# ltatzel/PyTorchHessianFree

Hardware: AMD Instinct MI355X
Metric: GGN-matvecs/sec (damped operator calls inside the PCG loop) (higher is better)
Workload: dtype f32

## Files before the change

include/hf_pcg.h:

```cpp
#ifndef HF_PCG_H
#define HF_PCG_H

#include <stdint.h>

#ifdef __cplusplus
extern "C" {
#endif

#define HF_ABI_VERSION 13

enum hf_dtype { HF_F32 = 0, HF_F64 = 1 };

enum hf_reason {
  HF_RUNNING = 0,
  HF_REASON_MARTENS = 1,
  HF_REASON_MAXITER = 2,
  HF_REASON_DIVERGED = 3,
  HF_REASON_TOL = 4
};

enum hf_precond {
  HF_M_NONE = 0,
  HF_M_DIAG = 1,
  HF_M_EXTERNAL = 2
// ... 229 lines not shown
int hf_maxpool_forward_nhwc(void* out, void* out2, int64_t out2_ld, void* idx, const void* x, int64_t n,
                            int64_t h, int64_t w, int64_t oh, int64_t ow, int64_t c, int64_t kh, int64_t kw,
                            int64_t stride_h, int64_t stride_w, int64_t pad_h, int64_t pad_w, int dtype,
                            void* stream);
int hf_maxpool_adjoint_nhwc(void* g, const void* gy_a, int a_splits, int64_t a_slab, const void* gy_b,
                            int b_splits, int64_t b_slab, const void* idx, int64_t n, int64_t h, int64_t w,
                            int64_t oh, int64_t ow, int64_t c, int64_t kh, int64_t kw, int64_t stride_h,
                            int64_t stride_w, int64_t pad_h, int64_t pad_w, int dtype, void* stream);
int hf_linear_ce_head(void* g_feat, void* g_w, void* g_b, const void* t_feat, const void* feat, const void* w,
                      const void* v_w, const void* v_b, const void* p, double scale, int64_t rows,
                      int64_t features, int64_t classes, int dtype, void* stream);
int hf_linear_ce_head_slabs(int64_t rows);
int hf_pool_ce_head(void* g, void* jv_out, const void* t, const void* p, double scale, int64_t n, int64_t hw,
                    int64_t k, int dtype, void* stream);

typedef struct hf_comm hf_comm_t;
int hf_comm_unique_id(char* out128);
int hf_comm_create(hf_comm_t** out, const char* id128, int nranks, int rank);
int hf_comm_destroy(hf_comm_t* c);
int hf_allreduce_sum(hf_comm_t* c, void* buf, int64_t n, int dtype, void* stream);
int hf_allreduce_sum_multi(hf_comm_t* c, void* const* bufs, const int64_t* ns, int count, int dtype,
                           void* stream);

#ifdef __cplusplus
}
#endif
#endif
```

pytorchhessianfree_amd/_lib.py:

```python

import ctypes
import os

import torch

_HERE = os.path.dirname(os.path.abspath(__file__))
LIB_PATH = os.environ.get("HF_PCG_LIB") or os.path.join(_HERE, "csrc", "libhfpcg.so")

HF_F32, HF_F64 = 0, 1
ABI_VERSION = 13
HF_ERR_ARG = -1
HF_M_NONE, HF_M_DIAG, HF_M_EXTERNAL = 0, 1, 2
REASONS = {
    1: "Convergence (Martens)",
    2: "Number of iterations",
    3: "Divergence",
    4: "Convergence (tolerances)",
}

c_void_p, c_int, c_int64, c_double = (
    ctypes.c_void_p,
    ctypes.c_int,
    ctypes.c_int64,
    ctypes.c_double,
)
# ... 75 lines not shown
                                                  c_int, c_void_p]),
    "hf_chan_affine_bwd": (c_int, [c_void_p] * 11 + [c_int64, c_int64, c_int64, c_int, c_int, c_void_p]),
    "hf_conv2d_nhwc": (c_int, [c_int, c_void_p, c_void_p, c_void_p] + [c_int64] * 12
                       + [c_void_p, c_int64, c_void_p, c_int64, c_int, c_int, c_void_p]),
    "hf_conv2d_nhwc_backward": (c_int, [c_void_p] * 5 + [c_int64] * 11
                                + [c_void_p, c_int64, c_void_p, c_int64, c_int, c_int, c_void_p]),
    "hf_conv2d_nhwc_plan": (c_int, [c_int] + [c_int64] * 11 + [c_int]),
    "hf_conv2d_nhwc_slabs": (c_int, [c_int, c_void_p, c_void_p, c_void_p] + [c_int64] * 14
                             + [c_int, c_int64, c_int, c_void_p]),
    "hf_conv2d_nhwc_slabs_unpack": (c_int, [c_void_p, c_void_p, c_void_p] + [c_int64] * 13 + [c_int, c_int64, c_void_p,
                                            ctypes.POINTER(c_void_p)] + [ctypes.POINTER(c_int64)] * 6
                                    + [c_int, c_int, c_void_p]),
    "hf_conv2d_nhwc_group_slabs": (c_int, [c_void_p, c_int, c_int, c_void_p]),
    "hf_conv2d_nhwc_dw_slabs": (c_int, [c_void_p, c_void_p, c_int, c_void_p]),
    "hf_chan_affine_pair": (c_int, [c_void_p, c_int, c_void_p]),
    "hf_chan_affine_bwd_pair": (c_int, [c_void_p, c_int, c_void_p]),
    "hf_conv2d_nhwc_backward_slabs": (c_int, [c_void_p] * 5 + [c_int64] * 11
                                      + [c_int, c_int64, c_int, c_int64, c_int, c_void_p]),
    "hf_chan_affine_ex": (c_int, [c_void_p] * 10 + [c_int, c_int64, c_int64, c_int64, c_int, c_int64, c_int64,
                                                     c_int, c_int64, c_int, c_void_p]),
    "hf_chan_affine_bwd_ex": (c_int, [c_void_p] * 5 + [c_int, c_int64, c_void_p, c_int, c_int64] + [c_void_p] * 5
                              + [c_int64, c_int64, c_int64, c_int, c_int, c_int, c_void_p]),
    "hf_chan_affine_train": (c_int, [c_void_p] * 8 + [c_int, c_void_p, c_void_p, c_double, c_void_p, c_void_p]
                             + [c_int64] * 5 + [c_int, c_int64, c_int, c_void_p]),
    "hf_conv2d_nhwc_group_slabs_bnsum": (c_int, [c_void_p, c_int, c_void_p, c_int, c_void_p]),
    "hf_bn_forward_train": (c_int, [c_void_p, c_void_p, c_int64, c_void_p, c_void_p, c_int] + [c_void_p] * 4
                            + [c_double] * 3 + [c_void_p] * 3 + [c_int64, c_int, c_int64, c_int64, c_int, c_void_p]),
    "hf_chan_affine_train_pair": (c_int, [c_void_p, c_int, c_void_p]),
    "hf_bn_train_hessian_coeffs": (c_int, [c_void_p] * 5 + [c_int, c_void_p, c_void_p, c_int] + [c_void_p] * 5
                                   + [c_double, c_int64, c_int, c_void_p]),
# ... 285 lines not shown
    check(
        lib.hf_pack_ex(c_void_p(dst.data_ptr()), ptrs, numels, perm, spl, lv, n, float(scale), int(mode),
                       dtype_code(dst.dtype), current_stream_ptr(dst.device)),
        "hf_pack_ex")
    return dst


class AffineProblem(ctypes.Structure):

    _fields_ = ([("out", c_void_p)] + [(nm, c_void_p) for nm in ("a", "x", "mean", "rstd", "w", "q", "r", "add",
                                                                   "mask_src")]
                + [("relu_self", c_int)] + [(nm, c_int64) for nm in ("n", "c", "hw", "out_ld", "add_ld")]
                + [("a_splits", c_int), ("a_slab", c_int64)])


class BnAdjointProblem(ctypes.Structure):

    _fields_ = ([(nm, c_void_p) for nm in ("gx", "gw", "gb", "gres", "gy")] + [("gy_splits", c_int), ("gy_slab", c_int64),
                                                                                 ("gy2", c_void_p), ("gy2_splits", c_int),
                                                                                 ("gy2_slab", c_int64)]
                + [(nm, c_void_p) for nm in ("x", "mean", "rstd", "w", "mask_src")]
                + [(nm, c_int64) for nm in ("n", "c", "hw")] + [("row_blocks", c_int)])


class AffineTrainProblem(ctypes.Structure):

    _fields_ = ([("out", c_void_p)] + [(nm, c_void_p) for nm in ("a", "x", "mean", "rstd", "w", "part_x", "part_1")]
                + [("nparts", c_int), ("vq", c_void_p), ("vr", c_void_p), ("count", ctypes.c_double),
                   ("add", c_void_p), ("mask_src", c_void_p)]
                + [(nm, c_int64) for nm in ("n", "c", "hw", "out_ld")] + [("a_splits", c_int), ("a_slab", c_int64)])
# ... 85 lines not shown
```

pytorchhessianfree_amd/config.py:

```python

import os
import shutil
import tempfile

_SHIPPED_DB = os.path.join(os.path.dirname(os.path.abspath(__file__)), "miopen_db")
_state = {"done": False, "settings": None}


def user_db_dir():
    base = os.environ.get("XDG_CACHE_HOME") or os.path.join(os.path.expanduser("~"), ".cache")
    return os.path.join(base, "pytorchhessianfree_amd", "miopen_db")


def _seed_user_db(dst):
    os.makedirs(dst, exist_ok=True)
    for name in sorted(os.listdir(_SHIPPED_DB)):
        src, out = os.path.join(_SHIPPED_DB, name), os.path.join(dst, name)
        if not os.path.isfile(src) or os.path.exists(out):
            continue
        fd, tmp = tempfile.mkstemp(dir=dst, prefix=name + ".")
        os.close(fd)
        try:
            shutil.copyfile(src, tmp)
            os.replace(tmp, out)
# ... 52 lines not shown
                "tests/test_optimizer_gpu.py::test_deterministic_mode_products_are_bitwise_repeatable"),
    "HF_NHWC_FIND": ("", "1: keep MIOpen's find step for NHWC problems (used once to produce the shipped records)",
                     "tests/test_host_logic_cpu.py::test_configure_is_explicit_and_idempotent"),
    "HF_SESSION": ("1", "0: no persistent engine session (engine + graphs rebuilt per step)",
                   "tests/test_session_gpu.py::test_session_equals_generic_path_and_is_faster_to_restart"),
    "HF_SESSION_VERIFY": ("", "1: re-verify the session against the model's own forward pass every step",
                          "tests/test_session_gpu.py::test_session_is_reverified_against_the_models_own_forward"),
    "HF_SESSION_VERIFY_EVERY": ("16", "every how many steps the session is re-verified",
                                "tests/test_session_gpu.py::test_session_is_reverified_against_the_models_own_forward"),
    "HF_ACC_SESSION": ("1", "0: acc_step on the generic accumulation",
                       "tests/test_acc_session_gpu.py::test_acc_step_train_mode_batchnorm_session_equals_generic_accumulation"),
    "HF_GRAPH_VERIFY": ("first", "always / never: replay check of a freshly captured product graph",
                        "tests/test_optimizer_gpu.py::test_graphed_operator_refuses_a_replay_that_differs_from_the_eager_product"),
    "HF_FUSE_ITERATION": ("1", "0: product, K1, K2, K3 as separate launches (no iteration graph)",
                          "tests/test_engine_gpu.py::test_solve_as_one_graph_per_iteration_equals_separate_launches"),
    "HF_BN_EPILOGUE": ("1", "0: train-mode tangent partial sums by the reduction launch, not the convolution's epilogue",
                       "tests/test_engine_gpu.py::test_train_mode_prologue_form_variants_agree_and_state_is_independent_of_the_first_use_check"),
    "HF_BN_TRAIN_PAIR": ("1", "0: a downsample block's two train-mode units in launches of their own",
                         "tests/test_engine_gpu.py::test_train_mode_prologue_form_variants_agree_and_state_is_independent_of_the_first_use_check"),
    "HF_CHUNKED_ALLREDUCE": ("auto", "0 / 1: force the single-graph resp. the two-phase data-parallel product",
                             "tests/test_distributed_gpu.py::test_step_two_ranks_engine_session_equals_cpu_whole_batch"),
    "HF_DIRECT_RCCL": ("1", "0: every collective through torch.distributed (no communicator of the package's own)",
                       "tests/test_distributed_gpu.py::test_bench_ladder_reaches_the_plainest_rung"),
    "HF_TEST_DP_FAULT": ("", "test hook: hang / raise / mismatch[:not_plain] -- the last rank misbehaves in a data-parallel "
                             "session product (session._inject_fault)",
                         "tests/test_distributed_gpu.py::test_bench_ladder_falls_past_a_rung_that_hangs"),
    "HF_PCG_BLOCKS": ("0", "workgroups of the PCG vector kernels (0: 2 per CU); must agree on all ranks",
                      "tests/test_cg_gpu.py::test_kernel_grid_override_gives_the_same_solve"),
    "HF_PCG_LIB": ("", "path of another build of libhfpcg.so (tuning variants)",
                   "tests/test_boundary.py::test_alternate_library_path"),
# ... 7 lines not shown
```

pytorchhessianfree_amd/csrc/build.py:

```python

import os
import subprocess
import sys

HERE = os.path.dirname(os.path.abspath(__file__))
ROOT = os.path.dirname(os.path.dirname(HERE))
SOURCES = [os.path.join(HERE, f) for f in ("hf_pcg.hip", "hf_pack.hip", "hf_bn.hip", "hf_conv.hip", "hf_head.hip",
                                           "hf_rccl.hip")]
HDR = os.path.join(ROOT, "include", "hf_pcg.h")
HDRS_SHARED = [os.path.join(HERE, f) for f in ("hf_common.h", "hf_unpack.h")]
OUT = os.path.join(HERE, "libhfpcg.so")

FLAGS = [
    "--offload-arch=gfx950",
    "-O3",
    "-std=c++17",
    "-fPIC",
    "-ffp-contract=off",
    "-fno-fast-math",
    "-Wall",
    "-Wno-unused-function",
]


# ... 37 lines not shown
```

pytorchhessianfree_amd/engine/adjoint.py:

```python

import os

import torch

from .. import _lib
from .common import _cl, _pair, _ptr


class _AdjointSweep:
    def _bn_adjoint_pair_train(self, u1, srcs1, u2, srcs2):
        self._bn_adjoint_pair(u1, srcs1, u2, srcs2, train=True)
        arr = (_lib.AffineTrainProblem * 2)()
        for q, u in zip(arr, (u1, u2)):
            self._affine_train_problem(q, u, u.ga, 0, u.g, 1, 0, u.gw, u.gb, u.rb, None, None, None)
        _lib.check(_lib.load().hf_chan_affine_train_pair(_lib.ctypes.cast(arr, _lib.c_void_p), _lib.HF_F32,
                                                         _lib.current_stream_ptr(self.dev)), "hf_chan_affine_train_pair")

    def _bn_adjoint_pair(self, u1, srcs1, u2, srcs2, train=False):
        arr = (_lib.BnAdjointProblem * 2)()
        for q, u, srcs in zip(arr, (u1, u2), (srcs1, srcs2)):
            if not 1 <= len(srcs) <= 2:
                raise RuntimeError(f"{u.name}: {len(srcs)} consumers")
            (a, sa, la) = srcs[0]
            (b, sb, lb) = srcs[1] if len(srcs) == 2 else (None, 1, 0)
            n, k, oh, ow = u.a.shape
            q.gx, q.gw, q.gb, q.gres = (None if train else u.ga.data_ptr()), u.gw.data_ptr(), u.gb.data_ptr(), u.g.data_ptr()
            q.gy, q.gy_splits, q.gy_slab = a.data_ptr(), sa, la
            q.gy2, q.gy2_splits, q.gy2_slab = (None if b is None else b.data_ptr()), sb, lb
            q.x, q.mean, q.rstd, q.w = u.a.data_ptr(), u.mean.data_ptr(), u.rstd.data_ptr(), u.bn.weight.data_ptr()
            q.mask_src = u.y.data_ptr() if u.relu else None
            q.n, q.c, q.hw, q.row_blocks = n, k, oh * ow, u.rb
        _lib.check(_lib.load().hf_chan_affine_bwd_pair(_lib.ctypes.cast(arr, _lib.c_void_p), _lib.HF_F32,
                                                       _lib.current_stream_ptr(self.dev)), "hf_chan_affine_bwd_pair")

    def _adjoint_unit(self, u, srcs):
        second = self._second and u.bn is not None
        self._bn_adjoint(u, srcs, reduce_only=second and u.train)
        if not second:
            self._conv_adjoint(u)
            return
        lib, st = _lib.load(), _lib.current_stream_ptr(self.dev)
        n, k, oh, ow = u.a.shape
        v = self._v
        v_gamma = v[self._offs[u.pg]: self._offs[u.pg] + k] if u.pg is not None else self._zeros(k)
        if not self._extras_parallel:
            self._hessian_extras(u)
        if u.train:
            rb = u.rb
            tx, t1, nparts_t = u.tsums
            _lib.check(lib.hf_bn_train_hessian_coeffs(
# ... 62 lines not shown

    def _adjoint_blocks(self, g_last, first=None, last_block=0, incoming=None):
        group = self._grouping()
        tail = self.tail
        if incoming is None:
            incoming = {id(tail): [(g_last, 1, 0)]}
        pool_srcs = None
        first = len(self.blocks) - 1 if first is None else first
        stop = max(last_block, self.dead_blocks)
        for bi in range(first, stop - 1, -1):
            chain, ds, _x = self.blocks[bi]
            head, last = chain[0], chain[-1]
            for k in range(len(chain) - 1, -1, -1):
                u = chain[k]
                if k == 0 and ds is not None and group:
                    if u.rb > 1 and ds.rb > 1 and not u.train and not ds.train:
                        self._bn_adjoint_pair(u, incoming.pop(id(u)), ds, [(last.g, 1, 0)])
                    elif u.rb > 1 and ds.rb > 1 and self._train_pair_ok(u, ds):
                        self._bn_adjoint_pair_train(u, incoming.pop(id(u)), ds, [(last.g, 1, 0)])
                    else:
                        self._bn_adjoint(u, incoming.pop(id(u)))
                        self._bn_adjoint(ds, [(last.g, 1, 0)])
                    if u.no_dgrad:
                        _lib.conv_group_slabs(
                            [(2, u.wbuf, u.x, u.ga, u.geo, u.sW, 0, 0), (2, ds.wbuf, ds.x, ds.ga, ds.geo, ds.sW, 0, 0)],
                            self.dev)
                    else:
                        _lib.conv_group_slabs(
                            [(1, u.dbuf, u.ga, u.wT, u.geo, u.sD, 0, 0), (2, u.wbuf, u.x, u.ga, u.geo, u.sW, 0, 0),
                             (1, ds.dbuf, ds.ga, ds.wT, ds.geo, ds.sD, 0, 0),
# ... 124 lines not shown
```

pytorchhessianfree_amd/engine/buffers.py:

```python

import os

import torch
from torch import nn

from .. import _lib
from .common import _Unsupported, _flat_view, _live_taps, _pair, _ptr


class _Buffers:
    ADJ_BYTES_PER_WG = 32768
    def _plan(self, direction, u, forward=False):
        n, c, h, w = u.x.shape
        k, _, r, s = u.conv.weight.shape
        cin = 2 * c if (direction == 0 and not forward) else c
        sp = _lib.load().hf_conv2d_nhwc_plan(direction, n, h, w, cin, k, r, s, u.conv.stride[0], u.conv.stride[1],
                                             u.conv.padding[0], u.conv.padding[1],
                                             0)
        if sp < 1:
            raise _Unsupported(f"{u.name}: convolution geometry refused ({sp})")
        return sp

    def _allocate(self):
        dev, f32 = self.dev, torch.float32
        cl = torch.channels_last

        def nhwc(shape):
            return torch.empty(shape, dtype=f32, device=dev).contiguous(memory_format=cl)

        self._nhwc = nhwc
        self.x_in = nhwc(self._in_shape)
        if self.pool_args is not None:
            self.pool_out = nhwc(self.pool_out.shape)
        for u in self.units:
            u.a, u.y = nhwc(u.a.shape), nhwc(u.y.shape)
            if u.train:
                u.rstd_version = None
            elif u.bn is not None:
                u.rstd = torch.rsqrt(u.bn.running_var + u.bn.eps)
                u.rstd_version = u.bn.running_var._version
        tails = {id(c[-1]): c[0] for c, _, _ in self.blocks}
        for u in self.units:
            u.x = self.x_in if u.src == "input" else self.pool_out if u.src == "pool" else u.src.y
            if u.res_unit is not None:
                u.res = u.res_unit.y
            elif u.res_identity:
                u.res = tails[id(u)].x
            else:
                u.res = None
        xcats = {}
        self._tangent_slots = {}
        for u in self.units:
            n, c, h, w = u.x.shape
            k, _, r, s = u.conv.weight.shape
            if u.im2col:
                if c * r * s > 256:
                    raise _Unsupported(f"{u.name}: too many taps for the im2col formulation")
                oh, ow = u.a.shape[2], u.a.shape[3]
                j = c * r * s
                u.cols = torch.empty((n, oh * ow, j), dtype=f32, device=dev)
                u.geo = (n * oh * ow, 1, 1, j, k, 1, 1, (1, 1), (0, 0))
                jp = -(-j // 4) * 4
                u.cols_pad = torch.zeros((n, oh * ow, jp), dtype=f32, device=dev)
                u.geo_w = (n * oh * ow, 1, 1, jp, k, 1, 1, (1, 1), (0, 0))
# ... 11 lines not shown
                u.wcat = torch.zeros((k, 2 * c, r, s), dtype=f32, device=dev).contiguous(memory_format=cl)
                u.wT = torch.empty((c, r, s, k), dtype=f32, device=dev)
                u.live = _live_taps(h, w, r, s, u.conv.stride, u.conv.padding)
                if u.pw is not None:
                    self._tangent_slots[id(u)] = (self._offs[u.pw], u.wcat, c, u.live)
            oh, ow = u.a.shape[2], u.a.shape[3]
            u.rows, u.cout = n * oh * ow, k
            if u.im2col:
                u.sT = u.sF = self._plan_stem(0, u.geo)
                u.sW = self._plan_stem(2, u.geo_w)
                u.sD = 0
            else:
                u.sT, u.sW = self._plan(0, u), self._plan(2, u)
                u.sD = 0 if (u.first or u.no_dgrad or u.dead) else self._plan(1, u)
                u.sF = self._plan(0, u, forward=True)
            u.tbuf = torch.empty((max(u.sT, u.sF), u.rows * k), dtype=f32, device=dev)
            u.nW = u.sW * (2 if (self.hessian and not u.first) else 1)
            u.nD = u.sD * (2 if self.hessian else 1)
            u.wbuf = torch.zeros((u.nW, u.conv.weight.numel()), dtype=f32, device=dev)
            if u.sD:
                u.dbuf = torch.empty((u.nD, u.x.numel()), dtype=f32, device=dev)
            if self.hessian:
                u.ga1 = torch.empty_like(u.a)
                if u.bn is not None:
                    u.g1 = torch.empty_like(u.a)
                    u.gah = torch.empty_like(u.a)
                if u.sD:
                    u.vT = torch.zeros((c, r, s, k), dtype=f32, device=dev)
            u.g = torch.empty_like(u.a) if u.needs_g else None
            u.ga = torch.empty_like(u.a)
            u.rb = 1
            if k % 4 == 0 and k // 4 <= 256 and u.rows >= 64:
                rp = 256 // (k // 4)
                tgt = min(1024, max(64, u.a.numel() * 4 // self.ADJ_BYTES_PER_WG))
                per = max(rp, -(-u.rows // tgt))
                u.rb = -(-u.rows // per)
                if u.rb < 2:
                    u.rb = 1
            u.gw_rows = u.rb * (2 if (self.hessian and u.bn is not None) else 1)
            if self.hessian and u.train:
                u.gw_rows += 1
            u.gw = torch.empty((u.gw_rows, k), dtype=f32, device=dev)
            u.gb = torch.empty((u.rb, k), dtype=f32, device=dev)
            if u.train:
                if not (k % 4 == 0 and k // 4 <= 256):
                    raise _Unsupported(f"{u.name}: train-mode BatchNorm over {k} channels (the prologue form takes "
                                       "multiples of 4 up to 1024)")
                u.stat_part = torch.empty((u.rb, 2, k), dtype=torch.float64, device=dev)
                tp_rows = -(-u.rows // 64) * u.sT
                u.epi = (not u.im2col and not u.first and hasattr(u, "xcat")
                         and tp_rows <= 256
                         and os.environ.get("HF_BN_EPILOGUE", "1") != "0")
                if self.hessian:
# ... 161 lines not shown
```

pytorchhessianfree_amd/engine/common.py:

```python

import os

import torch

from .. import _lib

_P = _lib.c_void_p


def _ptr(t):
    return _P(t.data_ptr()) if t is not None else None


def _same(a, b):
    return a is not None and b is not None and a.data_ptr() == b.data_ptr() and a.shape == b.shape


def _cl(t):
    return t.contiguous(memory_format=torch.channels_last)


class _Unit:

    def __init__(self, name, conv, bn):
        self.name, self.conv, self.bn = name, conv, bn
        self.rstd = None
        self.first = False
        self.needs_g = True
        self.im2col = False
        self.train = False
        self.mean_t = None
        self.epi = self.tsum = False
        self.res_unit = None
        self.res_identity = False
        self.consumers = 0
        self.src = None
        self.dead = False
        self.no_dgrad = False

    @property
    def mean(self):
        if self.train:
            return self.mean_t
        return self.bn.running_mean if self.bn is not None else None

    @property
    def scale(self):
        return self.bn.weight if self.bn is not None else None

    @property
    def shift(self):
        return self.bn.bias if self.bn is not None else self.conv.bias

# ... 84 lines not shown
    if p0.dtype != torch.float32 or not p0.is_cuda:
        return None
    base, off = p0.data_ptr(), 0
    for p in params:
        if not p.is_contiguous() or p.data_ptr() != base + 4 * off or p.dtype != torch.float32:
            return None
        off += p.numel()
    try:
        if p0.untyped_storage().nbytes() < 4 * (p0.storage_offset() + n) or base % 16:
            return None
        return p0.detach().as_strided((n,), (1,), p0.storage_offset())
    except Exception:
        return None


def _live_taps(h, w, r, s, stride, padding):
    if r * s > 16:
        return 0
    oh = (h + 2 * padding[0] - r) // stride[0] + 1
    ow = (w + 2 * padding[1] - s) // stride[1] + 1
    rows = [any(0 <= o * stride[0] - padding[0] + i < h for o in range(oh)) for i in range(r)]
    cols = [any(0 <= o * stride[1] - padding[1] + j < w for o in range(ow)) for j in range(s)]
    mask = sum(1 << (i * s + j) for i in range(r) for j in range(s) if rows[i] and cols[j])
    return 0 if mask == (1 << (r * s)) - 1 else mask
```

pytorchhessianfree_amd/engine/tangent.py:

```python

import os

import torch

from .. import _lib
from .common import _ptr


class _TangentSweep:
    def _bn_tangent(self, u, v, add, add_ld):
        n, k, oh, ow = u.a.shape
        vg = v[self._offs[u.pg]: self._offs[u.pg] + k] if u.pg is not None else None
        vb = v[self._offs[u.pb]: self._offs[u.pb] + k] if u.pb is not None else None
        if u.train:
            lib, st = _lib.load(), _lib.current_stream_ptr(self.dev)
            px, p1, nparts = u.gw, u.gb, u.rb
            if self.hessian:
                px, p1 = u.hx, u.h1
                _lib.check(lib.hf_chan_affine_bwd_ex(
                    None, _ptr(u.gw[u.rb:]), None, None, _ptr(u.tbuf), u.sT, u.tbuf.shape[1], None, 1, 0, _ptr(u.g1),
                    _ptr(self._zeros(k)), _ptr(u.rstd), None, None, n, k, oh * ow, 1, u.rb, _lib.HF_F32, st),
                    "hf_chan_affine_bwd_ex")
            if u.tsum:
                px, p1, nparts = u.tpx, u.tp1, u.tp1.shape[0]
# ... 77 lines not shown
            sums = [(u.a, u.mean, u.rstd, u.tpx, u.tp1) if u.epi else None for u in units]
            if _lib.conv_group_slabs_bnsum(probs, sums, self.dev):
                for u in units:
                    u.tsum = u.epi
                return
            for u in units:
                u.epi = False
        for u in units:
            u.tsum = False
        if len(units) == 1:
            u = units[0]
            self._conv_slabs(0, u.tbuf, u.xcat, u.wcat, self._tgeo(u), u.sT)
        else:
            _lib.conv_group_slabs(probs, self.dev)

    def _tangent_blocks(self, v):
        group = self._grouping()
        for chain, ds, _x in self.blocks[self.dead_blocks:]:
            head = chain[0]
            paired = False
            if ds is not None and group:
                self._tangent_convs([ds, head])
                alone = head.res_unit is None and not head.res_identity and len(chain) > 1
                paired = alone and not head.train and not ds.train
                if paired:
                    self._bn_tangent_pair(ds, head, v)
                elif alone and self._train_pair_ok(ds, head) and ds.tsum and head.tsum:
                    self._bn_tangent_pair_train(ds, head, v)
                    paired = True
                else:
                    self._bn_tangent(ds, v, None, 0)
            elif ds is not None:
                self._tangent_convs([ds])
                self._bn_tangent(ds, v, None, 0)
            for u in chain:
                if u is head and paired:
                    continue
                if not (u is head and ds is not None and group):
                    self._tangent_convs([u])
                add, add_ld = None, 0
                if u.res_unit is not None:
                    add, add_ld = u.res_unit.tout, u.res_unit.tout_ld
                elif u.res_identity:
                    c = head.x.shape[1]
                    add, add_ld = head.xcat[:, :c], 2 * c
                self._bn_tangent(u, v, add, add_ld)

    def _head(self, v):
        tail = self.tail
        t_last = tail.tout
        hw = t_last.shape[2] * t_last.shape[3]
        fw = self.fc.weight
        nf = fw.numel()
        v_fw = v[self._offs[self.pfw]: self._offs[self.pfw] + nf].view_as(fw)
        v_fb = None if self.pfb is None else v[self._offs[self.pfb]: self._offs[self.pfb] + fw.shape[0]]
        if self.hessian:
            t_feat = t_last.flatten(1) if hw == 1 else t_last.mean(dim=(2, 3))
            if self.pfb is not None:
                Jv = torch.addmm(v_fb, t_feat, fw.detach().t())
            else:
# ... 53 lines not shown
```

Baseline: 1506.

## Add fused skinny MFMA kernels for units with a 1x1 output map

Adds a new HIP file with dedicated tangent and adjoint kernels for small-batch convolution units whose output spatial map is 1x1. Each kernel folds the tap-sparse GEMM (MFMA 16x16x4 f32), the batch-norm affine, the residual add and the ReLU mask into one launch. This replaces the generic split-K convolution plus separate elementwise launches in those layers. The Python engine marks eligible units, routes the tangent and adjoint passes through the new kernels, and reshapes split and reduction buffers to fit. The cost is new code paths with eligibility constraints; they are off for hessian and train mode.

```diff
diff --git a/include/hf_pcg.h b/include/hf_pcg.h
--- a/include/hf_pcg.h
+++ b/include/hf_pcg.h
@@ -7,7 +7,7 @@
 extern "C" {
 #endif
 
-#define HF_ABI_VERSION 13
+#define HF_ABI_VERSION 14
 
 enum hf_dtype { HF_F32 = 0, HF_F64 = 1 };
 
@@ -267,6 +267,28 @@
 int hf_pool_ce_head(void* g, void* jv_out, const void* t, const void* p, double scale, int64_t n, int64_t hw,
                     int64_t k, int dtype, void* stream);
 
+#define HF_SKINNY_MAX_TAPS 9
+#define HF_SKINNY_MAX_ROWS 64
+typedef struct hf_skinny_tangent_problem {
+  void* out;
+  const void *act, *mat, *x, *mean, *rstd, *w, *q, *r, *add, *mask_src;
+  int64_t rows, cout, kc, act_ld, mat_ld, out_ld, add_ld;
+  int ntaps;
+  int64_t act_off[HF_SKINNY_MAX_TAPS], mat_off[HF_SKINNY_MAX_TAPS];
+} hf_skinny_tangent_problem;
+int hf_skinny_tangent(const hf_skinny_tangent_problem* problems, int count, int dtype, void* stream);
+typedef struct hf_skinny_adjoint_problem {
+  const void *gy, *gy2, *mask_src, *w, *rstd, *a, *mean;
+  void *g, *ga, *gw, *gb, *dx;
+  const void* wT;
+  void* dw;
+  const void* x;
+  int64_t rows, cout, cin, npix, rs;
+  int ntaps;
+  int64_t tap_rs[HF_SKINNY_MAX_TAPS], tap_pix[HF_SKINNY_MAX_TAPS];
+} hf_skinny_adjoint_problem;
+int hf_skinny_adjoint(const hf_skinny_adjoint_problem* problems, int count, int dtype, void* stream);
+
 typedef struct hf_comm hf_comm_t;
 int hf_comm_unique_id(char* out128);
 int hf_comm_create(hf_comm_t** out, const char* id128, int nranks, int rank);
diff --git a/pytorchhessianfree_amd/_lib.py b/pytorchhessianfree_amd/_lib.py
--- a/pytorchhessianfree_amd/_lib.py
+++ b/pytorchhessianfree_amd/_lib.py
@@ -8,7 +8,7 @@
 LIB_PATH = os.environ.get("HF_PCG_LIB") or os.path.join(_HERE, "csrc", "libhfpcg.so")
 
 HF_F32, HF_F64 = 0, 1
-ABI_VERSION = 13
+ABI_VERSION = 14
 HF_ERR_ARG = -1
 HF_M_NONE, HF_M_DIAG, HF_M_EXTERNAL = 0, 1, 2
 REASONS = {
@@ -114,6 +114,8 @@
     "hf_conv2d_nhwc_group_slabs": (c_int, [c_void_p, c_int, c_int, c_void_p]),
     "hf_conv2d_nhwc_dw_slabs": (c_int, [c_void_p, c_void_p, c_int, c_void_p]),
     "hf_chan_affine_pair": (c_int, [c_void_p, c_int, c_void_p]),
+    "hf_skinny_tangent": (c_int, [c_void_p, c_int, c_int, c_void_p]),
+    "hf_skinny_adjoint": (c_int, [c_void_p, c_int, c_int, c_void_p]),
     "hf_chan_affine_bwd_pair": (c_int, [c_void_p, c_int, c_void_p]),
     "hf_conv2d_nhwc_backward_slabs": (c_int, [c_void_p] * 5 + [c_int64] * 11
                                       + [c_int, c_int64, c_int, c_int64, c_int, c_void_p]),
@@ -429,6 +431,25 @@
                 + [("a_splits", c_int), ("a_slab", c_int64)])
 
 
+SKINNY_MAX_TAPS, SKINNY_MAX_ROWS = 9, 64
+
+
+class SkinnyTangentProblem(ctypes.Structure):
+
+    _fields_ = ([("out", c_void_p)] + [(nm, c_void_p) for nm in ("act", "mat", "x", "mean", "rstd", "w", "q", "r", "add",
+                                                                   "mask_src")]
+                + [(nm, c_int64) for nm in ("rows", "cout", "kc", "act_ld", "mat_ld", "out_ld", "add_ld")]
+                + [("ntaps", c_int), ("act_off", c_int64 * SKINNY_MAX_TAPS), ("mat_off", c_int64 * SKINNY_MAX_TAPS)])
+
+
+class SkinnyAdjointProblem(ctypes.Structure):
+
+    _fields_ = ([(nm, c_void_p) for nm in ("gy", "gy2", "mask_src", "w", "rstd", "a", "mean", "g", "ga", "gw", "gb", "dx",
+                                           "wT", "dw", "x")]
+                + [(nm, c_int64) for nm in ("rows", "cout", "cin", "npix", "rs")]
+                + [("ntaps", c_int), ("tap_rs", c_int64 * SKINNY_MAX_TAPS), ("tap_pix", c_int64 * SKINNY_MAX_TAPS)])
+
+
 class BnAdjointProblem(ctypes.Structure):
 
     _fields_ = ([(nm, c_void_p) for nm in ("gx", "gw", "gb", "gres", "gy")] + [("gy_splits", c_int), ("gy_slab", c_int64),
diff --git a/pytorchhessianfree_amd/config.py b/pytorchhessianfree_amd/config.py
--- a/pytorchhessianfree_amd/config.py
+++ b/pytorchhessianfree_amd/config.py
@@ -90,6 +90,8 @@
                         "tests/test_optimizer_gpu.py::test_graphed_operator_refuses_a_replay_that_differs_from_the_eager_product"),
     "HF_FUSE_ITERATION": ("1", "0: product, K1, K2, K3 as separate launches (no iteration graph)",
                           "tests/test_engine_gpu.py::test_solve_as_one_graph_per_iteration_equals_separate_launches"),
+    "HF_SKINNY": ("1", "0: units with a 1x1 output map on the generic split-K convolution + elementwise launches",
+                  "tests/test_skinny_gpu.py::test_resnet18_product_skinny_equals_generic_path"),
     "HF_BN_EPILOGUE": ("1", "0: train-mode tangent partial sums by the reduction launch, not the convolution's epilogue",
                        "tests/test_engine_gpu.py::test_train_mode_prologue_form_variants_agree_and_state_is_independent_of_the_first_use_check"),
     "HF_BN_TRAIN_PAIR": ("1", "0: a downsample block's two train-mode units in launches of their own",
diff --git a/pytorchhessianfree_amd/csrc/build.py b/pytorchhessianfree_amd/csrc/build.py
--- a/pytorchhessianfree_amd/csrc/build.py
+++ b/pytorchhessianfree_amd/csrc/build.py
@@ -5,8 +5,8 @@
 
 HERE = os.path.dirname(os.path.abspath(__file__))
 ROOT = os.path.dirname(os.path.dirname(HERE))
-SOURCES = [os.path.join(HERE, f) for f in ("hf_pcg.hip", "hf_pack.hip", "hf_bn.hip", "hf_conv.hip", "hf_head.hip",
-                                           "hf_rccl.hip")]
+SOURCES = [os.path.join(HERE, f) for f in ("hf_pcg.hip", "hf_pack.hip", "hf_bn.hip", "hf_conv.hip", "hf_skinny.hip",
+                                           "hf_head.hip", "hf_rccl.hip")]
 HDR = os.path.join(ROOT, "include", "hf_pcg.h")
 HDRS_SHARED = [os.path.join(HERE, f) for f in ("hf_common.h", "hf_unpack.h")]
 OUT = os.path.join(HERE, "libhfpcg.so")
diff --git a/pytorchhessianfree_amd/csrc/hf_skinny.hip b/pytorchhessianfree_amd/csrc/hf_skinny.hip
--- /dev/null
+++ b/pytorchhessianfree_amd/csrc/hf_skinny.hip
@@ -0,0 +1,378 @@
+#include "hf_common.h"
+
+namespace {
+
+typedef float sk_f32x4 __attribute__((ext_vector_type(4)));
+struct alignas(16) SF4 { float e[4]; };
+
+constexpr int SK_WAVES = 8;
+constexpr int SK_BLOCK = SK_WAVES * 64;
+constexpr int SK_TAPS = HF_SKINNY_MAX_TAPS;
+constexpr int SK_ROWS = HF_SKINNY_MAX_ROWS;
+constexpr int SK_TAN_BATCH = 8;
+constexpr int SK_ADJ_BATCH = 2;
+
+__device__ __forceinline__ SF4 sk_ld4(const float* p) { return *reinterpret_cast<const SF4*>(p); }
+__device__ __forceinline__ SF4 sk_zero4() { SF4 z; z.e[0] = z.e[1] = z.e[2] = z.e[3] = 0.f; return z; }
+
+constexpr int SK_LD = 36;
+constexpr int SK_TILE = 16 * SK_LD;
+
+__device__ __forceinline__ void sk_wave_sync() {
+  __builtin_amdgcn_fence(__ATOMIC_ACQ_REL, "wavefront");
+  __builtin_amdgcn_wave_barrier();
+}
+
+__device__ __forceinline__ void sk_stage(float* tile, const SF4& lo, const SF4& hi, int lane) {
+  float* q = tile + (lane >> 3) * SK_LD + 4 * (lane & 7);
+  *reinterpret_cast<SF4*>(q) = lo;
+  *reinterpret_cast<SF4*>(q + 8 * SK_LD) = hi;
+}
+
+__device__ __forceinline__ void sk_mma_tiles(const float* ta, const float* tb, int lane, sk_f32x4& acc) {
+  const int m = lane & 15, kq = lane >> 4;
+#pragma unroll
+  for (int jj = 0; jj < 2; ++jj) {
+    const SF4 fa = sk_ld4(ta + m * SK_LD + 4 * (kq + 4 * jj)), fb = sk_ld4(tb + m * SK_LD + 4 * (kq + 4 * jj));
+#pragma unroll
+    for (int j = 0; j < 4; ++j) acc = __builtin_amdgcn_mfma_f32_16x16x4f32(fa.e[j], fb.e[j], acc, 0, 0, 0);
+  }
+}
+
+__device__ __forceinline__ float sk_reduce_tiles(const sk_f32x4& acc, float (*red)[256]) {
+  const int lane = threadIdx.x & 63, wave = threadIdx.x >> 6;
+#pragma unroll
+  for (int i = 0; i < 4; ++i) red[wave][i * 64 + lane] = acc[i];
+  __syncthreads();
+  float s = 0.f;
+  if (threadIdx.x < 256) {
+    s = red[0][threadIdx.x];
+#pragma unroll
+    for (int w = 1; w < SK_WAVES; ++w) s += red[w][threadIdx.x];
+  }
+  return s;
+}
+
+struct SkTanArgs {
+  float* out;
+  const float *act, *mat;
+  const float *x, *mean, *rstd, *w, *q, *r, *add, *mask;
+  int rows, cout, kc, ntaps, col_tiles, blocks;
+  unsigned act_ld, mat_ld, out_ld, add_ld;
+  int act_off[SK_TAPS], mat_off[SK_TAPS];
+};
+
+__device__ __forceinline__ void sk_tangent_body(const SkTanArgs& p, int bid, float (*red)[256], float* stage) {
+  const int lane = threadIdx.x & 63, wave = threadIdx.x >> 6;
+  const int lr = lane >> 3, lk = 4 * (lane & 7);
+  const int ct = bid % p.col_tiles, rt = bid / p.col_tiles;
+  const bool ok0 = rt * 16 + lr < p.rows, ok1 = rt * 16 + 8 + lr < p.rows;
+  const float* arow0 = p.act + (size_t)(ok0 ? rt * 16 + lr : 0) * p.act_ld + lk;
+  const float* arow1 = p.act + (size_t)(ok1 ? rt * 16 + 8 + lr : 0) * p.act_ld + lk;
+  const float* brow0 = p.mat + (size_t)(ct * 16 + lr) * p.mat_ld + lk;
+  const float* brow1 = brow0 + (size_t)8 * p.mat_ld;
+  float *ta = stage + wave * 2 * SK_TILE, *tb = ta + SK_TILE;
+  const int per_tap = p.kc >> 5, chunks = p.ntaps * per_tap;
+  sk_f32x4 acc = {0.f, 0.f, 0.f, 0.f};
+  for (int base = wave; base < chunks; base += SK_TAN_BATCH * SK_WAVES) {
+    SF4 a0[SK_TAN_BATCH], a1[SK_TAN_BATCH], b0[SK_TAN_BATCH], b1[SK_TAN_BATCH];
+#pragma unroll
+    for (int u = 0; u < SK_TAN_BATCH; ++u) {
+      const int ch = base + u * SK_WAVES < chunks ? base + u * SK_WAVES : base;
+      const int t = ch / per_tap, kk = (ch - t * per_tap) << 5;
+      const int ao = p.act_off[t] + kk, bo = p.mat_off[t] + kk;
+      a0[u] = sk_ld4(arow0 + ao), a1[u] = sk_ld4(arow1 + ao), b0[u] = sk_ld4(brow0 + bo), b1[u] = sk_ld4(brow1 + bo);
+    }
+#pragma unroll
+    for (int u = 0; u < SK_TAN_BATCH; ++u) {
+      if (base + u * SK_WAVES < chunks) {
+        sk_stage(ta, ok0 ? a0[u] : sk_zero4(), ok1 ? a1[u] : sk_zero4(), lane);
+        sk_stage(tb, b0[u], b1[u], lane);
+        sk_wave_sync();
+        sk_mma_tiles(ta, tb, lane, acc);
+        sk_wave_sync();
+      }
+    }
+  }
+  const float s = sk_reduce_tiles(acc, red);
+  if (threadIdx.x >= 256) return;
+  const int orow = rt * 16 + 4 * (lane >> 4) + (threadIdx.x >> 6), c = ct * 16 + (lane & 15);
+  if (orow >= p.rows) return;
+  const size_t i = (size_t)orow * p.cout + c;
+  const float rs = p.rstd ? p.rstd[c] : 1.f;
+  float v = s * ((p.w ? p.w[c] : 1.f) * rs);
+  if (p.q) v += ((p.x[i] - p.mean[c]) * rs) * p.q[c];
+  if (p.r) v += p.r[c];
+  if (p.add) v += p.add[p.add_ld ? (size_t)orow * p.add_ld + c : i];
+  if (p.mask) v = p.mask[i] > 0.f ? v : 0.f;
+  p.out[p.out_ld ? (size_t)orow * p.out_ld + c : i] = v;
+}
+
+__global__ __launch_bounds__(SK_BLOCK) void k_skinny_tangent(const SkTanArgs A, const SkTanArgs B) {
+  __shared__ float red[SK_WAVES][256];
+  __shared__ alignas(16) float stage[SK_WAVES * 2 * SK_TILE];
+  if ((int)blockIdx.x < A.blocks) sk_tangent_body(A, blockIdx.x, red, stage);
+  else sk_tangent_body(B, blockIdx.x - A.blocks, red, stage);
+}
+
+struct SkAdjArgs {
+  const float *gy, *gy2, *mask, *w, *rstd, *a, *mean;
+  float *g, *ga, *gw, *gb;
+  float* dx;
+  const float* wT;
+  float* dw;
+  const float* x;
+  int rows, cout, cin, npix, rs, ntaps;
+  int row_tiles, d_col_tiles, d_blocks, w_col_groups, blocks;
+  int tap_rs[SK_TAPS], tap_pix[SK_TAPS], pix_tap[SK_TAPS];
+};
+
+__device__ __forceinline__ void sk_cot4(const SkAdjArgs& p, bool row_ok, int row, int k, SF4& g, SF4& ga) {
+  const size_t i = (size_t)(row_ok ? row : 0) * p.cout + k;
+  SF4 h = sk_zero4(), m = sk_zero4(), w4 = sk_zero4(), rs4 = sk_zero4();
+  g = sk_ld4(p.gy + i);
+  if (p.gy2) h = sk_ld4(p.gy2 + i);
+  if (p.mask) m = sk_ld4(p.mask + i);
+  if (p.w) w4 = sk_ld4(p.w + k);
+  if (p.rstd) rs4 = sk_ld4(p.rstd + k);
+#pragma unroll
+  for (int j = 0; j < 4; ++j) {
+    float gg = g.e[j];
+    if (p.gy2) gg = gg + h.e[j];
+    if (p.mask) gg = m.e[j] > 0.f ? gg : 0.f;
+    gg = row_ok ? gg : 0.f;
+    const float s = (p.w ? w4.e[j] : 1.f) * (p.rstd ? rs4.e[j] : 1.f);
+    g.e[j] = gg;
+    ga.e[j] = gg * s;
+  }
+}
+
+__device__ __forceinline__ float sk_cot1(const SkAdjArgs& p, int row, int k) {
+  const bool row_ok = row < p.rows;
+  const size_t i = (size_t)(row_ok ? row : 0) * p.cout + k;
+  float gg = p.gy[i];
+  if (p.gy2) gg = gg + p.gy2[i];
+  if (p.mask) gg = p.mask[i] > 0.f ? gg : 0.f;
+  gg = row_ok ? gg : 0.f;
+  const float s = (p.w ? p.w[k] : 1.f) * (p.rstd ? p.rstd[k] : 1.f);
+  return gg * s;
+}
+
+__device__ __forceinline__ double sk_rowsum16(double lo, double hi) {
+  double v = lo + hi;
+#pragma unroll
+  for (int off = 8; off < 64; off <<= 1) v += __shfl_xor(v, off, 64);
+  return v;
+}
+
+__device__ __forceinline__ void sk_adj_publish(const SkAdjArgs& p, bool ok0, bool ok1, int row, int rt, int lane, int k,
+                                               const SF4& g0, const SF4& ga0, const SF4& g1, const SF4& ga1) {
+  const size_t i0 = (size_t)(ok0 ? row : 0) * p.cout + k, i1 = (size_t)(ok1 ? row + 8 : 0) * p.cout + k;
+  if (ok0) {
+    if (p.g) *reinterpret_cast<SF4*>(p.g + i0) = g0;
+    *reinterpret_cast<SF4*>(p.ga + i0) = ga0;
+  }
+  if (ok1) {
+    if (p.g) *reinterpret_cast<SF4*>(p.g + i1) = g1;
+    *reinterpret_cast<SF4*>(p.ga + i1) = ga1;
+  }
+  if (!p.gw && !p.gb) return;
+  SF4 x0 = sk_zero4(), x1 = sk_zero4(), mu = sk_zero4(), rs4 = sk_zero4();
+  if (p.gw) {
+    x0 = sk_ld4(p.a + i0), x1 = sk_ld4(p.a + i1);
+    mu = sk_ld4(p.mean + k);
+    rs4 = sk_ld4(p.rstd + k);
+  }
+  SF4 sw, sb;
+#pragma unroll
+  for (int j = 0; j < 4; ++j) {
+    const double d0 = (double)g0.e[j] * (double)(float)((x0.e[j] - mu.e[j]) * rs4.e[j]);
+    const double d1 = (double)g1.e[j] * (double)(float)((x1.e[j] - mu.e[j]) * rs4.e[j]);
+    sw.e[j] = (float)sk_rowsum16(ok0 ? d0 : 0.0, ok1 ? d1 : 0.0);
+    sb.e[j] = (float)sk_rowsum16((double)g0.e[j], (double)g1.e[j]);
+  }
+  if (lane < 8) {
+    if (p.gw) *reinterpret_cast<SF4*>(p.gw + (size_t)rt * p.cout + k) = sw;
+    if (p.gb) *reinterpret_cast<SF4*>(p.gb + (size_t)rt * p.cout + k) = sb;
+  }
+}
+
+__device__ __forceinline__ void sk_adjoint_body(const SkAdjArgs& p, int bid, float (*red)[256], float* stage) {
+  const int lane = threadIdx.x & 63, wave = threadIdx.x >> 6;
+  const int m = lane & 15, kq = lane >> 4;
+  if (bid < p.d_blocks) {
+    const int ct = bid % p.d_col_tiles, rt = bid / p.d_col_tiles;
+    const int lr = lane >> 3, lk = 4 * (lane & 7);
+    const int row = rt * 16 + lr;
+    const bool ok0 = row < p.rows, ok1 = row + 8 < p.rows;
+    const bool publish = ct == 0;
+    const bool dgrad = p.dx != nullptr;
+    const int j0 = ct * 16, pix = j0 / p.cin, c0 = j0 - pix * p.cin;
+    const int tap = dgrad ? p.pix_tap[pix] : -1;
+    if (!publish && tap < 0) {
+      if (dgrad && threadIdx.x < 256) {
+        const int orow = rt * 16 + 4 * (lane >> 4) + (threadIdx.x >> 6);
+        if (orow < p.rows) p.dx[((size_t)orow * p.npix + pix) * p.cin + c0 + (lane & 15)] = 0.f;
+      }
+      return;
+    }
+    const float* brow0 = tap < 0 ? nullptr : p.wT + ((size_t)(c0 + lr) * p.rs + p.tap_rs[tap]) * p.cout + lk;
+    const float* brow1 = tap < 0 ? nullptr : brow0 + (size_t)8 * p.rs * p.cout;
+    float *ta = stage + wave * 2 * SK_TILE, *tb = ta + SK_TILE;
+    const int chunks = p.cout >> 5;
+    sk_f32x4 acc = {0.f, 0.f, 0.f, 0.f};
+    for (int base = wave; base < chunks; base += SK_ADJ_BATCH * SK_WAVES) {
+      SF4 g0[SK_ADJ_BATCH], g1[SK_ADJ_BATCH], a0[SK_ADJ_BATCH], a1[SK_ADJ_BATCH], b0[SK_ADJ_BATCH], b1[SK_ADJ_BATCH];
+#pragma unroll
+      for (int u = 0; u < SK_ADJ_BATCH; ++u) {
+        const int kk = (base + u * SK_WAVES < chunks ? base + u * SK_WAVES : base) << 5;
+        b0[u] = b1[u] = sk_zero4();
+        if (brow0) { b0[u] = sk_ld4(brow0 + kk); b1[u] = sk_ld4(brow1 + kk); }
+        sk_cot4(p, ok0, row, kk + lk, g0[u], a0[u]);
+        sk_cot4(p, ok1, row + 8, kk + lk, g1[u], a1[u]);
+      }
+#pragma unroll
+      for (int u = 0; u < SK_ADJ_BATCH; ++u) {
+        if (base + u * SK_WAVES < chunks) {
+          const int kk = (base + u * SK_WAVES) << 5;
+          if (publish) sk_adj_publish(p, ok0, ok1, row, rt, lane, kk + lk, g0[u], a0[u], g1[u], a1[u]);
+          sk_stage(ta, a0[u], a1[u], lane);
+          sk_stage(tb, b0[u], b1[u], lane);
+          sk_wave_sync();
+          sk_mma_tiles(ta, tb, lane, acc);
+          sk_wave_sync();
+        }
+      }
+    }
+    if (!dgrad) return;
+    const float s = sk_reduce_tiles(acc, red);
+    if (threadIdx.x >= 256) return;
+    const int orow = rt * 16 + 4 * (lane >> 4) + (threadIdx.x >> 6);
+    if (orow < p.rows) p.dx[((size_t)orow * p.npix + pix) * p.cin + c0 + (lane & 15)] = tap < 0 ? 0.f : s;
+    return;
+  }
+  bid -= p.d_blocks;
+  const int kt = bid / p.w_col_groups, cg = bid - kt * p.w_col_groups;
+  const int groups_per_tap = p.cin >> 7;
+  const int t = cg / groups_per_tap, c0 = ((cg - t * groups_per_tap) << 7) + wave * 16;
+  const float* xcol = p.x + (size_t)p.tap_pix[t] * p.cin + c0 + m;
+  const size_t xrow = (size_t)p.npix * p.cin;
+  const int k = kt * 16 + m;
+  sk_f32x4 acc = {0.f, 0.f, 0.f, 0.f};
+  float av[SK_ROWS / 4], bv[SK_ROWS / 4];
+#pragma unroll
+  for (int s = 0; s < SK_ROWS / 4; ++s) {
+    const int n = 4 * s + kq;
+    av[s] = bv[s] = 0.f;
+    if (4 * s < p.rows) {
+      av[s] = sk_cot1(p, n, k);
+      const float xv = xcol[(size_t)(n < p.rows ? n : 0) * xrow];
+      bv[s] = n < p.rows ? xv : 0.f;
+    }
+  }
+#pragma unroll
+  for (int s = 0; s < SK_ROWS / 4; ++s)
+    if (4 * s < p.rows) acc = __builtin_amdgcn_mfma_f32_16x16x4f32(av[s], bv[s], acc, 0, 0, 0);
+  float* o = p.dw + ((size_t)(kt * 16 + 4 * kq) * p.rs + p.tap_rs[t]) * p.cin + c0 + m;
+#pragma unroll
+  for (int i = 0; i < 4; ++i) o[(size_t)i * p.rs * p.cin] = acc[i];
+}
+
+__global__ __launch_bounds__(SK_BLOCK) void k_skinny_adjoint(const SkAdjArgs A, const SkAdjArgs B) {
+  __shared__ float red[SK_WAVES][256];
+  __shared__ alignas(16) float stage[SK_WAVES * 2 * SK_TILE];
+  if ((int)blockIdx.x < A.blocks) sk_adjoint_body(A, blockIdx.x, red, stage);
+  else sk_adjoint_body(B, blockIdx.x - A.blocks, red, stage);
+}
+
+bool sk_fill_tangent(SkTanArgs& a, const hf_skinny_tangent_problem& q) {
+  if (!q.out || !q.act || !q.mat || q.rows < 1 || q.rows > SK_ROWS || q.cout < 16 || q.cout % 16 || q.kc < 32 ||
+      q.kc % 32 || q.ntaps < 1 || q.ntaps > SK_TAPS)
+    return false;
+  if ((q.q && (!q.x || !q.mean || !q.rstd)) || (q.out_ld && q.out_ld < q.cout) || (q.add_ld && (q.add_ld < q.cout || !q.add)))
+    return false;
+  if (q.act_ld % 4 || q.mat_ld % 4 || !aligned16(q.act) || !aligned16(q.mat) || q.act_ld > 0x3fffffffLL ||
+      q.mat_ld > 0x3fffffffLL || q.out_ld > 0x3fffffffLL || q.add_ld > 0x3fffffffLL)
+    return false;
+  a.out = (float*)q.out;
+  a.act = (const float*)q.act, a.mat = (const float*)q.mat;
+  a.x = (const float*)q.x, a.mean = (const float*)q.mean, a.rstd = (const float*)q.rstd, a.w = (const float*)q.w;
+  a.q = (const float*)q.q, a.r = (const float*)q.r, a.add = (const float*)q.add, a.mask = (const float*)q.mask_src;
+  a.rows = (int)q.rows, a.cout = (int)q.cout, a.kc = (int)q.kc, a.ntaps = q.ntaps;
+  a.col_tiles = a.cout / 16;
+  a.blocks = a.col_tiles * ((a.rows + 15) / 16);
+  a.act_ld = (unsigned)q.act_ld, a.mat_ld = (unsigned)q.mat_ld, a.out_ld = (unsigned)q.out_ld, a.add_ld = (unsigned)q.add_ld;
+  for (int t = 0; t < SK_TAPS; ++t) {
+    a.act_off[t] = a.mat_off[t] = 0;
+    if (t < q.ntaps) {
+      if (q.act_off[t] < 0 || q.mat_off[t] < 0 || q.act_off[t] % 4 || q.mat_off[t] % 4 ||
+          q.act_off[t] + q.kc > q.act_ld || q.mat_off[t] + q.kc > q.mat_ld)
+        return false;
+      a.act_off[t] = (int)q.act_off[t], a.mat_off[t] = (int)q.mat_off[t];
+    }
+  }
+  return true;
+}
+
+}
+
+extern "C" {
+
+int hf_skinny_tangent(const hf_skinny_tangent_problem* problems, int count, int dtype, void* stream) {
+  if (!problems || count < 1 || count > 2 || dtype != HF_F32) return HF_ERR_ARG;
+  SkTanArgs a[2];
+  memset(a, 0, sizeof(a));
+  for (int i = 0; i < count; ++i)
+    if (!sk_fill_tangent(a[i], problems[i])) return HF_ERR_ARG;
+  const int blocks = a[0].blocks + (count == 2 ? a[1].blocks : 0);
+  hipLaunchKernelGGL(k_skinny_tangent, dim3(blocks), dim3(SK_BLOCK), 0, (hipStream_t)stream, a[0], a[1]);
+  HF_HIP(hipGetLastError());
+  return HF_OK;
+}
+
+static int sk_fill_adjoint(SkAdjArgs& a, const hf_skinny_adjoint_problem* q) {
+  if (!q->gy || !q->ga || !q->dw || !q->x || q->rows < 1 || q->rows > SK_ROWS || q->cout < 32 || q->cout % 32 ||
+      q->cin < 128 || q->cin % 128 || q->npix < 1 || q->npix > SK_TAPS || q->rs < 1 || q->ntaps < 1 ||
+      q->ntaps > SK_TAPS || q->ntaps > q->rs)
+    return HF_ERR_ARG;
+  if ((q->gw && (!q->a || !q->mean || !q->rstd)) || (q->dx && !q->wT)) return HF_ERR_ARG;
+  const void* al[] = {q->gy, q->gy2, q->mask_src, q->w, q->rstd, q->a, q->mean, q->g, q->ga, q->gw, q->gb, q->dx,
+                      q->wT, q->dw, q->x};
+  for (const void* ptr : al)
+    if (!aligned16(ptr)) return HF_ERR_ALIGN;
+  a.gy = (const float*)q->gy, a.gy2 = (const float*)q->gy2, a.mask = (const float*)q->mask_src;
+  a.w = (const float*)q->w, a.rstd = (const float*)q->rstd, a.a = (const float*)q->a, a.mean = (const float*)q->mean;
+  a.g = (float*)q->g, a.ga = (float*)q->ga, a.gw = (float*)q->gw, a.gb = (float*)q->gb;
+  a.dx = (float*)q->dx, a.wT = (const float*)q->wT, a.dw = (float*)q->dw, a.x = (const float*)q->x;
+  a.rows = (int)q->rows, a.cout = (int)q->cout, a.cin = (int)q->cin, a.npix = (int)q->npix, a.rs = (int)q->rs;
+  a.ntaps = q->ntaps;
+  for (int t = 0; t < SK_TAPS; ++t) a.pix_tap[t] = -1;
+  for (int t = 0; t < q->ntaps; ++t) {
+    if (q->tap_rs[t] < 0 || q->tap_rs[t] >= q->rs || q->tap_pix[t] < 0 || q->tap_pix[t] >= q->npix) return HF_ERR_ARG;
+    if (a.pix_tap[q->tap_pix[t]] >= 0) return HF_ERR_ARG;
+    a.tap_rs[t] = (int)q->tap_rs[t], a.tap_pix[t] = (int)q->tap_pix[t];
+    a.pix_tap[a.tap_pix[t]] = t;
+  }
+  a.row_tiles = (a.rows + 15) / 16;
+  a.d_col_tiles = a.dx ? a.npix * a.cin / 16 : 1;
+  a.d_blocks = a.d_col_tiles * a.row_tiles;
+  a.w_col_groups = a.ntaps * (a.cin / 128);
+  a.blocks = a.d_blocks + (a.cout / 16) * a.w_col_groups;
+  return HF_OK;
+}
+
+int hf_skinny_adjoint(const hf_skinny_adjoint_problem* problems, int count, int dtype, void* stream) {
+  if (!problems || count < 1 || count > 2 || dtype != HF_F32) return HF_ERR_ARG;
+  SkAdjArgs a[2];
+  memset(a, 0, sizeof(a));
+  for (int i = 0; i < count; ++i) {
+    const int rc = sk_fill_adjoint(a[i], problems + i);
+    if (rc) return rc;
+  }
+  const int blocks = a[0].blocks + (count == 2 ? a[1].blocks : 0);
+  hipLaunchKernelGGL(k_skinny_adjoint, dim3(blocks), dim3(SK_BLOCK), 0, (hipStream_t)stream, a[0], a[1]);
+  HF_HIP(hipGetLastError());
+  return HF_OK;
+}
+
+}
diff --git a/pytorchhessianfree_amd/engine/adjoint.py b/pytorchhessianfree_amd/engine/adjoint.py
--- a/pytorchhessianfree_amd/engine/adjoint.py
+++ b/pytorchhessianfree_amd/engine/adjoint.py
@@ -33,7 +33,31 @@
         _lib.check(_lib.load().hf_chan_affine_bwd_pair(_lib.ctypes.cast(arr, _lib.c_void_p), _lib.HF_F32,
                                                        _lib.current_stream_ptr(self.dev)), "hf_chan_affine_bwd_pair")
 
+    def _skinny_adjoint(self, items):
+        arr = (_lib.SkinnyAdjointProblem * len(items))()
+        for q, (u, srcs) in zip(arr, items):
+            if not 1 <= len(srcs) <= 2 or any(sp != 1 for _t, sp, _l in srcs):
+                raise RuntimeError(f"{u.name}: the cotangents of a 1x1 map arrive as {[sp for _t, sp, _l in srcs]} slabs")
+            self._extras_wait(srcs)
+            n, c, h, w = u.x.shape
+            k, _, r, s = u.conv.weight.shape
+            q.gy, q.gy2 = srcs[0][0].data_ptr(), (srcs[1][0].data_ptr() if len(srcs) == 2 else None)
+            q.mask_src, q.w, q.rstd = (u.y.data_ptr() if u.relu else None), u.scale.data_ptr(), u.rstd.data_ptr()
+            q.a, q.mean = u.a.data_ptr(), u.mean.data_ptr()
+            q.g, q.ga = (u.g.data_ptr() if u.needs_g else None), u.ga.data_ptr()
+            q.gw, q.gb = u.gw.data_ptr(), (u.gb.data_ptr() if u.pb is not None else None)
+            q.dx, q.wT = (u.dbuf.data_ptr() if u.sD else None), u.wT.data_ptr()
+            q.dw, q.x = u.wbuf.data_ptr(), u.x.data_ptr()
+            q.rows, q.cout, q.cin, q.npix, q.rs, q.ntaps = n, k, c, h * w, r * s, len(u.taps)
+            for t, (rs_, pix) in enumerate(u.taps):
+                q.tap_rs[t], q.tap_pix[t] = rs_, pix
+        _lib.check(_lib.load().hf_skinny_adjoint(_lib.ctypes.cast(arr, _lib.c_void_p), len(items), _lib.HF_F32,
+                                                 _lib.current_stream_ptr(self.dev)), "hf_skinny_adjoint")
+
     def _adjoint_unit(self, u, srcs):
+        if u.skinny:
+            self._skinny_adjoint([(u, srcs)])
+            return
         second = self._second and u.bn is not None
         self._bn_adjoint(u, srcs, reduce_only=second and u.train)
         if not second:
@@ -126,6 +150,13 @@
             for k in range(len(chain) - 1, -1, -1):
                 u = chain[k]
                 if k == 0 and ds is not None and group:
+                    if u.skinny and ds.skinny:
+                        self._skinny_adjoint([(u, incoming.pop(id(u))), (ds, [(last.g, 1, 0)])])
+                        continue
+                    if u.skinny or ds.skinny:
+                        self._adjoint_unit(u, incoming.pop(id(u)))
+                        self._adjoint_unit(ds, [(last.g, 1, 0)])
+                        continue
                     if u.rb > 1 and ds.rb > 1 and not u.train and not ds.train:
                         self._bn_adjoint_pair(u, incoming.pop(id(u)), ds, [(last.g, 1, 0)])
                     elif u.rb > 1 and ds.rb > 1 and self._train_pair_ok(u, ds):
diff --git a/pytorchhessianfree_amd/engine/buffers.py b/pytorchhessianfree_amd/engine/buffers.py
--- a/pytorchhessianfree_amd/engine/buffers.py
+++ b/pytorchhessianfree_amd/engine/buffers.py
@@ -5,7 +5,7 @@
 from torch import nn
 
 from .. import _lib
-from .common import _Unsupported, _flat_view, _live_taps, _pair, _ptr
+from .common import _Unsupported, _flat_view, _live_taps, _pair, _ptr, _skinny_taps
 
 
 class _Buffers:
@@ -21,6 +21,26 @@
             raise _Unsupported(f"{u.name}: convolution geometry refused ({sp})")
         return sp
 
+    def _mark_skinny(self):
+        for u in self.units:
+            u.skinny, u.taps = False, ()
+        if os.environ.get("HF_SKINNY", "1") == "0" or self.hessian or not self.blocks:
+            return
+
+        def eligible(u):
+            n, c, h, w = u.x.shape
+            k = u.a.shape[1]
+            return (not u.im2col and not u.first and not u.train and not u.dead and u.bn is not None
+                    and n <= _lib.SKINNY_MAX_ROWS and c % 128 == 0 and k % 32 == 0
+                    and h * w <= _lib.SKINNY_MAX_TAPS and tuple(u.conv.dilation) == (1, 1))
+
+        small = [u for u in self.units if tuple(u.a.shape[2:]) == (1, 1)]
+        if small and all(eligible(u) for u in small):
+            for u in small:
+                n, c, h, w = u.x.shape
+                _k, _c, r, s = u.conv.weight.shape
+                u.skinny, u.taps = True, _skinny_taps(h, w, r, s, tuple(u.conv.padding))
+
     def _allocate(self):
         dev, f32 = self.dev, torch.float32
         cl = torch.channels_last
@@ -48,6 +68,7 @@
                 u.res = tails[id(u)].x
             else:
                 u.res = None
+        self._mark_skinny()
         xcats = {}
         self._tangent_slots = {}
         for u in self.units:
@@ -89,6 +110,8 @@
                 u.sT, u.sW = self._plan(0, u), self._plan(2, u)
                 u.sD = 0 if (u.first or u.no_dgrad or u.dead) else self._plan(1, u)
                 u.sF = self._plan(0, u, forward=True)
+                if u.skinny:
+                    u.sW, u.sD = 1, min(u.sD, 1)
             u.tbuf = torch.empty((max(u.sT, u.sF), u.rows * k), dtype=f32, device=dev)
             u.nW = u.sW * (2 if (self.hessian and not u.first) else 1)
             u.nD = u.sD * (2 if self.hessian else 1)
@@ -112,6 +135,8 @@
                 u.rb = -(-u.rows // per)
                 if u.rb < 2:
                     u.rb = 1
+            if u.skinny:
+                u.rb = -(-u.rows // 16)
             u.gw_rows = u.rb * (2 if (self.hessian and u.bn is not None) else 1)
             if self.hessian and u.train:
                 u.gw_rows += 1
diff --git a/pytorchhessianfree_amd/engine/common.py b/pytorchhessianfree_amd/engine/common.py
--- a/pytorchhessianfree_amd/engine/common.py
+++ b/pytorchhessianfree_amd/engine/common.py
@@ -37,6 +37,8 @@
         self.src = None
         self.dead = False
         self.no_dgrad = False
+        self.skinny = False
+        self.taps = ()
 
     @property
     def mean(self):
@@ -151,6 +153,11 @@
         return None
 
 
+def _skinny_taps(h, w, r, s, padding):
+    return tuple((i * s + j, (i - padding[0]) * w + (j - padding[1])) for i in range(r) for j in range(s)
+                 if 0 <= i - padding[0] < h and 0 <= j - padding[1] < w)
+
+
 def _live_taps(h, w, r, s, stride, padding):
     if r * s > 16:
         return 0
diff --git a/pytorchhessianfree_amd/engine/tangent.py b/pytorchhessianfree_amd/engine/tangent.py
--- a/pytorchhessianfree_amd/engine/tangent.py
+++ b/pytorchhessianfree_amd/engine/tangent.py
@@ -115,12 +115,32 @@
         else:
             _lib.conv_group_slabs(probs, self.dev)
 
+    def _skinny_tangent(self, items, v):
+        arr = (_lib.SkinnyTangentProblem * len(items))()
+        for q, (u, add, add_ld) in zip(arr, items):
+            n, c, h, w = u.x.shape
+            k, _, r, s = u.conv.weight.shape
+            q.out, q.act, q.mat, q.x = u.tout.data_ptr(), u.xcat.data_ptr(), u.wcat.data_ptr(), u.a.data_ptr()
+            q.mean, q.rstd, q.w = u.mean.data_ptr(), u.rstd.data_ptr(), u.scale.data_ptr()
+            q.q = v.data_ptr() + 4 * self._offs[u.pg] if u.pg is not None else None
+            q.r = v.data_ptr() + 4 * self._offs[u.pb] if u.pb is not None else None
+            q.add, q.mask_src = (add.data_ptr() if add is not None else None), (u.y.data_ptr() if u.relu else None)
+            q.rows, q.cout, q.kc, q.act_ld, q.mat_ld = n, k, 2 * c, h * w * 2 * c, r * s * 2 * c
+            q.out_ld, q.add_ld, q.ntaps = u.tout_ld, add_ld, len(u.taps)
+            for t, (rs_, pix) in enumerate(u.taps):
+                q.act_off[t], q.mat_off[t] = pix * 2 * c, rs_ * 2 * c
+        _lib.check(_lib.load().hf_skinny_tangent(_lib.ctypes.cast(arr, _lib.c_void_p), len(items), _lib.HF_F32,
+                                                 _lib.current_stream_ptr(self.dev)), "hf_skinny_tangent")
+
     def _tangent_blocks(self, v):
         group = self._grouping()
         for chain, ds, _x in self.blocks[self.dead_blocks:]:
             head = chain[0]
             paired = False
-            if ds is not None and group:
+            if ds is not None and ds.skinny:
+                paired = head.skinny and head.res_unit is None and not head.res_identity and len(chain) > 1
+                self._skinny_tangent([(ds, None, 0)] + ([(head, None, 0)] if paired else []), v)
+            elif ds is not None and group:
                 self._tangent_convs([ds, head])
                 alone = head.res_unit is None and not head.res_identity and len(chain) > 1
                 paired = alone and not head.train and not ds.train
@@ -137,14 +157,17 @@
             for u in chain:
                 if u is head and paired:
                     continue
-                if not (u is head and ds is not None and group):
-                    self._tangent_convs([u])
                 add, add_ld = None, 0
                 if u.res_unit is not None:
                     add, add_ld = u.res_unit.tout, u.res_unit.tout_ld
                 elif u.res_identity:
                     c = head.x.shape[1]
                     add, add_ld = head.xcat[:, :c], 2 * c
+                if u.skinny:
+                    self._skinny_tangent([(u, add, add_ld)], v)
+                    continue
+                if not (u is head and ds is not None and group and not ds.skinny):
+                    self._tangent_convs([u])
                 self._bn_tangent(u, v, add, add_ld)
 
     def _head(self, v):
```

Result: faster. 1558, median of 6 (+3.5%).
